# senikm/trpx

Hardware: AMD Instinct MI355X
Metric: frames/s (Terse encode + Prolix decode round trip, 512x512 uint16 stack, bit-exact vs CPU ref) (higher is better)
Workload: dtype u16

## Files before the change

### trpx_amd/csrc/encode_fused.hip

```cpp
#include <stddef.h>
#include <utility>
#include "codec_common.hpp"
#include "launchers.hpp"
#include "profile.hpp"
#include <stdlib.h>
#include <mutex>
#include <vector>

namespace trpx {

template <typename T> constexpr int sub_tiles() { return sizeof(T) <= 2 ? 4 : 5; }
template <typename T> constexpr int fused_occupancy() { return sizeof(T) <= 2 ? 8 : 4; }
[[maybe_unused]] constexpr uint64_t kWaitTicks = 25u * 1000u * 1000u;
struct SpinGuard {
    uint64_t t0 = 0;
    uint32_t spins = 0;
    __device__ __forceinline__ bool expired() {
#ifdef TRPX_FORCE_TIMEOUT
        return true;
#else
        if ((++spins & 63u) != 0u) return false;
        const uint64_t now = __builtin_amdgcn_s_memrealtime();
        if (t0 == 0) { t0 = now; return false; }
        return now - t0 > kWaitTicks;
#endif
    }
};

#ifdef TRPX_DIAGNOSTICS
#define TRPX_DIAG(a) ((a).debug)
#else
#define TRPX_DIAG(a) 0u
#endif

constexpr uint64_t kStInvalid = 0, kStAgg = 1, kStPrefix = 2;
constexpr uint32_t kGridY = 32768;
constexpr int kWmaxShift = 56;
constexpr uint64_t kBndHead = 1ull << 55;
constexpr uint64_t kHeadFlag = 1ull << 63, kTailFlag = 1ull << 62;
__device__ __forceinline__ uint64_t make_desc(uint64_t st, uint64_t v) { return (st << 62) | (v & ((1ull << 62) - 1)); }
__device__ __forceinline__ uint64_t desc_status(uint64_t d) { return d >> 62; }
__device__ __forceinline__ uint64_t desc_value(uint64_t d) { return d & ((1ull << 62) - 1); }

__device__ __forceinline__ uint64_t ld_desc(const uint64_t* p) {
    return __hip_atomic_load(p, __ATOMIC_RELAXED, __HIP_MEMORY_SCOPE_AGENT);
}
__device__ __forceinline__ void st_desc(uint64_t* p, uint64_t v) {
    __hip_atomic_store(p, v, __ATOMIC_RELAXED, __HIP_MEMORY_SCOPE_AGENT);
}

__device__ __forceinline__ uint64_t wave_sum64(uint64_t v) {
    const uint32_t l0 = (uint32_t)v & 0x1FFFFFu, l1 = (uint32_t)(v >> 21) & 0x1FFFFFu, l2 = (uint32_t)(v >> 42);
    const uint32_t s0 = (uint32_t)__builtin_amdgcn_readlane((int)wave_inclusive_scan(l0), 63);
    const uint32_t s1 = (uint32_t)__builtin_amdgcn_readlane((int)wave_inclusive_scan(l1), 63);
    const uint32_t s2 = (uint32_t)__builtin_amdgcn_readlane((int)wave_inclusive_scan(l2), 63);
    return (uint64_t)s0 + ((uint64_t)s1 << 21) + ((uint64_t)s2 << 42);
}

__device__ bool lookback(const uint64_t* __restrict__ desc, int64_t idx, int64_t lo, uint64_t* result) {
    const int lane = lane_id();
    uint64_t acc = 0;
    int64_t pos = idx - 1;
    while (pos >= lo) {
        const int64_t my = pos - lane;
        const bool in = my >= lo;
        uint64_t g = in ? 0ull : make_desc(kStPrefix, 0);
        uint32_t first_p = 64;
        SpinGuard guard;
        uint64_t need = ~0ull;
        for (;;) {
            if (desc_status(g) == kStInvalid && ((need >> lane) & 1ull)) g = ld_desc(desc + my);
            const uint64_t pmask = __ballot(desc_status(g) == kStPrefix);
            const uint64_t imask = __ballot(desc_status(g) == kStInvalid);
            first_p = pmask ? (uint32_t)__builtin_ctzll(pmask) : 64u;
            need = first_p >= 63u ? ~0ull : ((2ull << first_p) - 1ull);
            if ((imask & need) == 0) break;
            if (guard.expired()) return false;
            __builtin_amdgcn_s_sleep(2);
        }
        acc += wave_sum64((uint32_t)lane <= first_p ? desc_value(g) : 0ull);
        if (first_p < 64u) break;
        pos -= 64;
    }
    *result = acc;
    return true;
}

constexpr int kAccShift = 40;
constexpr uint32_t kAccLines = 2;
__host__ __device__ inline uint32_t fused_acc_lines(uint32_t tiles_per_frame) {
    const uint32_t k = (tiles_per_frame + 31u) / 32u;
    return k < 1u ? 1u : (k > kAccLines ? kAccLines : k);
}
constexpr uint64_t kPrefFlag = 1ull << 63;
__device__ bool lookback_frames(const uint64_t* __restrict__ acc_w, const uint64_t* __restrict__ pref_w, int64_t frame,
                                uint64_t tiles_per_frame, uint64_t* result, uint64_t stride, uint32_t n_acc) {
    const int lane = lane_id();
    uint64_t acc = 0;
    int64_t pos = frame - 1;
    while (pos >= 0) {
        const int64_t my = pos - lane;
        const bool in = my >= 0;
        uint64_t p = in ? 0ull : kPrefFlag, c = 0;
        uint32_t first_p = 64;
        SpinGuard guard;
        uint64_t need = ~0ull;
        bool complete = false;
        for (;;) {
            if (in && !(p & kPrefFlag) && !complete && ((need >> lane) & 1ull)) {
                p = ld_desc(pref_w + my * stride);
                c = ld_desc(acc_w + my * stride);
                for (uint32_t k = 1; k < n_acc; ++k) c += ld_desc(acc_w + my * stride + 16u * k);
                complete = (c >> kAccShift) == tiles_per_frame;
            }
            const uint64_t pmask = __ballot((p & kPrefFlag) != 0);
            const uint64_t cmask = __ballot(complete);
            first_p = pmask ? (uint32_t)__builtin_ctzll(pmask) : 64u;
            need = first_p >= 64u ? ~0ull : ((1ull << first_p) - 1ull);
            if ((~cmask & need) == 0) break;
            if (guard.expired()) return false;
            __builtin_amdgcn_s_sleep(2);
        }
        const uint64_t mine = (uint32_t)lane < first_p ? 1 + (c & ((1ull << kAccShift) - 1)) / 8
                                                       : ((uint32_t)lane == first_p ? p & ~kPrefFlag : 0ull);
        acc += wave_sum64(mine);
        if (first_p < 64u) break;
        pos -= 64;
    }
    *result = acc;
    return true;
}

template <typename T> struct Raw {
    static constexpr int bits = PixelTraits<T>::bits;
    static constexpr int per = 32 / bits;
    static constexpr int dw = kBlock / per;
};

template <typename T>
__device__ __forceinline__ uint32_t raw_field(const uint32_t (&raw)[Raw<T>::dw], int k) {
    constexpr int per = Raw<T>::per, bits = Raw<T>::bits;
    const uint32_t x = raw[k / per] >> ((k % per) * bits);
    return bits == 32 ? x : x & ((1u << (bits & 31)) - 1u);
}

template <typename T> struct QuadVec;
template <> struct QuadVec<uint8_t>  { typedef uint32_t type; };
template <> struct QuadVec<int8_t>   { typedef uint32_t type; };
template <> struct QuadVec<uint16_t> { typedef uint32_t type __attribute__((ext_vector_type(2))); };
template <> struct QuadVec<int16_t>  { typedef uint32_t type __attribute__((ext_vector_type(2))); };
template <> struct QuadVec<uint32_t> { typedef uint32_t type __attribute__((ext_vector_type(4))); };
template <> struct QuadVec<int32_t>  { typedef uint32_t type __attribute__((ext_vector_type(4))); };

template <typename T>
__device__ __forceinline__ void load_raw_nt(const T* __restrict__ p, uint32_t (&raw)[Raw<T>::dw]) {
    if constexpr (sizeof(T) == 2) {
        typedef uint32_t u4 __attribute__((ext_vector_type(4)));
        typedef uint32_t u2 __attribute__((ext_vector_type(2)));
        u4 lo; u2 hi;
        __builtin_memcpy(&lo, p, 16);
        __builtin_memcpy(&hi, reinterpret_cast<const char*>(p) + 16, 8);
        raw[0] = lo.x; raw[1] = lo.y; raw[2] = lo.z; raw[3] = lo.w; raw[4] = hi.x; raw[5] = hi.y;
        return;
    } else if constexpr (sizeof(T) == 1) {
        typedef uint32_t u3 __attribute__((ext_vector_type(3)));
        u3 x;
        __builtin_memcpy(&x, p, 12);
        raw[0] = x.x; raw[1] = x.y; raw[2] = x.z;
        return;
    }
    using V = typename QuadVec<T>::type;
    constexpr int q = Raw<T>::dw / 3;
    const V* src = reinterpret_cast<const V*>(p);
    union U { V vec; uint32_t x[q]; };
    U a, b, c;
    a.vec = src[0];
    b.vec = src[1];
    c.vec = src[2];
#pragma unroll
    for (int i = 0; i < q; ++i) { raw[i] = a.x[i]; raw[q + i] = b.x[i]; raw[2 * q + i] = c.x[i]; }
}
template <typename T>
__device__ __forceinline__ void load_raw_mis2(const T* __restrict__ p, uint32_t (&raw)[Raw<T>::dw]) {
    static_assert(sizeof(T) == 2, "16-bit pixels");
    typedef uint32_t u4 __attribute__((ext_vector_type(4)));
    typedef uint32_t u2 __attribute__((ext_vector_type(2)));
    const char* q = reinterpret_cast<const char*>(p) - 2;
    u4 lo; u2 hi; uint16_t last;
    __builtin_memcpy(&lo, q, 16);
    __builtin_memcpy(&hi, q + 16, 8);
    __builtin_memcpy(&last, q + 24, 2);
    raw[0] = __builtin_amdgcn_alignbit(lo.y, lo.x, 16); raw[1] = __builtin_amdgcn_alignbit(lo.z, lo.y, 16);
    raw[2] = __builtin_amdgcn_alignbit(lo.w, lo.z, 16); raw[3] = __builtin_amdgcn_alignbit(hi.x, lo.w, 16);
    raw[4] = __builtin_amdgcn_alignbit(hi.y, hi.x, 16); raw[5] = __builtin_amdgcn_alignbit((uint32_t)last, hi.y, 16);
}
template <typename T>
__device__ __forceinline__ void load_raw_partial(const T* __restrict__ p, int nb, uint32_t (&raw)[Raw<T>::dw]) {
    using UT = typename PixelTraits<T>::U;
#pragma unroll
    for (int i = 0; i < Raw<T>::dw; ++i) raw[i] = 0;
#pragma unroll
    for (int k = 0; k < kBlock; ++k)
        if (k < nb) raw[k / Raw<T>::per] |= (uint32_t)(UT)p[k] << ((k % Raw<T>::per) * Raw<T>::bits);
}

template <typename T>
__device__ __forceinline__ uint32_t raw_width(const uint32_t (&raw)[Raw<T>::dw]) {
    constexpr int bits = Raw<T>::bits;
    uint32_t m = 0;
    if (!PixelTraits<T>::is_signed) {
#pragma unroll
        for (int i = 0; i < Raw<T>::dw; ++i) m |= raw[i];
        if (bits == 16) m = (m | (m >> 16)) & 0xFFFFu;
        if (bits == 8) { m |= m >> 16; m = (m | (m >> 8)) & 0xFFu; }
    } else if (bits == 32) {
#pragma unroll
        for (int i = 0; i < Raw<T>::dw; ++i) {
            const uint32_t u = raw[i];
            m |= (int32_t)u < 0 ? 0u - u : u;
        }
    } else if (bits == 16) {
        typedef short s2 __attribute__((ext_vector_type(2)));
        typedef unsigned short us2 __attribute__((ext_vector_type(2)));
        uint32_t acc = 0;
#pragma unroll
        for (int i = 0; i < Raw<T>::dw; ++i) {
            union { uint32_t u; s2 v; us2 w; } x, n, y;
            x.u = raw[i];
            n.w = (us2)(0) - x.w;
            y.v = __builtin_elementwise_max(x.v, n.v);
            acc |= y.u;
        }
        m = (acc | (acc >> 16)) & 0xFFFFu;
    } else {
#pragma unroll
        for (int k = 0; k < kBlock; ++k) {
            const int32_t x = (int32_t)(int8_t)(raw[k / 4] >> ((k % 4) * 8));
            m |= (uint32_t)(x < 0 ? -x : x);
        }
    }
    return width_from_or<T>(m);
}

template <int ND>
__device__ __forceinline__ void lds_or_string(uint32_t* __restrict__ stage, uint32_t pos, uint32_t hv_top,
                                              const uint32_t* __restrict__ p) {
    const uint32_t d = (pos + 31u) >> 5, rs = (0u - pos) & 31u;
    const uint32_t xm = __builtin_amdgcn_alignbit(hv_top, 0u, rs);
    if (xm) atomicOr(&stage[d - 1], xm);
    if constexpr (ND == 0) {
        const uint32_t x0 = __builtin_amdgcn_alignbit(0u, hv_top, rs);
        if (x0) atomicOr(&stage[d], x0);
    } else {
        atomicOr(&stage[d], __builtin_amdgcn_alignbit(p[0], hv_top, rs));
#pragma unroll
        for (int j = 1; j < ND; ++j) {
            const uint32_t x = __builtin_amdgcn_alignbit(p[j], p[j - 1], rs);
            if (j >= ND - 1) atomicOr(&stage[d + j], x);
            else stage[d + j] = x;
        }
        const uint32_t x = __builtin_amdgcn_alignbit(0u, p[ND - 1], rs);
        if (x) atomicOr(&stage[d + ND], x);
    }
}

template <typename T, int W>
__device__ __forceinline__ void pack_payload_w(uint32_t* __restrict__ stage, uint32_t pos, uint32_t hv_top,
                                               const uint32_t (&raw)[Raw<T>::dw]) {
    constexpr int NB = kBlock * W;
    constexpr int ND = (NB + 31) / 32;
    constexpr int per = Raw<T>::per, bits = Raw<T>::bits;
    constexpr uint32_t MASK = W >= 32 ? 0xFFFFFFFFu : ((1u << (W & 31)) - 1u);
    uint32_t p[ND ? ND : 1];
#pragma unroll
    for (int j = 0; j < ND; ++j) p[j] = 0;
    if constexpr (W == 0) {
    } else if constexpr (bits == 16 && W < 16) {
        typedef unsigned short us2 __attribute__((ext_vector_type(2)));
        constexpr int L = (15 - W) / (2 * W) + 1;
        constexpr uint32_t kPairMask = MASK | (MASK << 16);
#pragma unroll
        for (int c = 0; c * L < kBlock / 2; ++c) {
            uint32_t acc = 0;
            int n_pairs = 0;
#pragma unroll
            for (int i = 0; i < L; ++i) {
                const int j = c * L + i;
                if (j < kBlock / 2) {
                    union { uint32_t u; us2 v; } x, k;
                    x.u = PixelTraits<T>::is_signed ? raw[j] & kPairMask : raw[j];
                    k.u = (1u << (2 * W * i)) | (1u << (2 * W * i + W + 16));
                    acc = __builtin_amdgcn_udot2(x.v, k.v, acc, false);
                    ++n_pairs;
                }
            }
            const int bit = 2 * W * L * c, nbits = 2 * W * n_pairs;
            p[bit >> 5] |= acc << (bit & 31);
            if ((bit & 31) + nbits > 32) p[(bit >> 5) + 1] |= acc >> (32 - (bit & 31));
        }
    } else if constexpr (bits == 16) {
#pragma unroll
        for (int j = 0; j < kBlock / 2; ++j) p[j] = raw[j];
    } else {
#pragma unroll
        for (int k = 0; k < kBlock; ++k) {
            const uint32_t u = (raw[k / per] >> ((k % per) * bits)) & MASK;
            const int bit = k * W;
            p[bit >> 5] |= u << (bit & 31);
            if ((bit & 31) + W > 32) p[(bit >> 5) + 1] |= u >> (32 - (bit & 31));
        }
    }
    lds_or_string<ND>(stage, pos, hv_top, p);
}

template <typename T, int LO, int HI>
struct PackDispatch {
    static __device__ __forceinline__ void run(uint32_t* stage, uint32_t pos, uint32_t hv_top, uint32_t w0,
                                               const uint32_t (&raw)[Raw<T>::dw]) {
        if constexpr (LO == HI) pack_payload_w<T, LO>(stage, pos, hv_top, raw);
        else {
            constexpr int MID = (LO + HI) / 2;
            if (w0 <= (uint32_t)MID) PackDispatch<T, LO, MID>::run(stage, pos, hv_top, w0, raw);
            else PackDispatch<T, MID + 1, HI>::run(stage, pos, hv_top, w0, raw);
        }
    }
};

template <typename T>
__device__ __forceinline__ void pack_payload_generic(uint32_t* __restrict__ stage, uint32_t pos, uint32_t w, int nb,
                                                     const uint32_t (&raw)[Raw<T>::dw]) {
    const uint32_t mask = w >= 32u ? 0xFFFFFFFFu : ((1u << w) - 1u);
#pragma unroll
    for (int k = 0; k < kBlock; ++k) {
        if (k < nb) {
            const uint64_t x = (uint64_t)(raw_field<T>(raw, k) & mask) << (pos & 31u);
            if ((uint32_t)x) atomicOr(&stage[pos >> 5], (uint32_t)x);
            if ((uint32_t)(x >> 32)) atomicOr(&stage[(pos >> 5) + 1], (uint32_t)(x >> 32));
            pos += w;
        }
    }
}

template <typename T> constexpr int fused_phase_rounds() { return (sub_tiles<T>() + 1) / 2; }
template <typename T>
constexpr int fused_stage_dwords() { return fused_phase_rounds<T>() * ((kThreads * max_block_bits<T>() + 31) / 32) + 12; }

struct FusedArgs {
    FrameGeom g;
    uint32_t n_frames;
    uint32_t tiles_per_frame;
    uint64_t out_capacity;
    uint64_t* tile_desc;
    uint64_t* tail_desc;
    uint64_t* bnd_pos;
    uint64_t* frame_acc;
    uint64_t* frame_pref;
    uint64_t* frame_base;
    uint32_t acc_stride;
    uint32_t n_acc;
    uint64_t* ws_tag;
    uint64_t expect_tag;
    uint64_t* frame_offsets;
    uint32_t* out32;
    uint32_t* status;
    uint8_t* idx_widths;
    uint64_t* idx_group_off;
    uint32_t debug;
    uint64_t* stamps;
};

typedef const char __attribute__((address_space(4)))* karg_ptr;
#define TRPX_KARG(kb, field) (*reinterpret_cast<const decltype(FusedArgs::field) __attribute__((address_space(4)))*>((kb) + 8 + offsetof(FusedArgs, field)))

template <typename T, bool MIS2>
__device__ __forceinline__ void encode_fused_body(const T* __restrict__ pixels, const FusedArgs& a) {
    constexpr int kSub = sub_tiles<T>();
    constexpr int kFusedTileBlocks = kSub * kThreads;
    constexpr int kStage = fused_stage_dwords<T>();
    constexpr int kStage4 = (kStage + 1 + 3) / 4;
    __shared__ __attribute__((aligned(16))) uint32_t s_stage_pad[4 * kStage4];
    uint32_t* const s_stage = s_stage_pad + 1;
    __shared__ uint32_t s_hdr[40];
    __shared__ uint32_t s_wtot[kSub * 4];
    __shared__ uint32_t s_wfl[kSub * 4];
    __shared__ uint64_t s_excl_bits;
    __shared__ uint64_t s_base_bytes;
    __shared__ uint32_t s_abort;
    __shared__ uint32_t s_carry;
    __shared__ uint32_t s_halo;

    const uint32_t tid = threadIdx.x;
#define TRPX_STAMP(slot) do { if ((TRPX_DIAG(a) & 4u) && threadIdx.x == 0) a.stamps[((uint64_t)(blockIdx.z * kGridY + blockIdx.y) * gridDim.x + blockIdx.x) * 8 + (slot)] = __builtin_amdgcn_s_memrealtime(); } while (0)
    TRPX_STAMP(0);
    const int lane = lane_id(), wave = wave_id();
    const FrameGeom g = a.g;
    const uint32_t t = blockIdx.x;
    const uint32_t frame = blockIdx.z * kGridY + blockIdx.y;
    const uint32_t n_frames = a.n_frames, tpf = a.tiles_per_frame;
    asm volatile("" :: "s"(g.n_values), "s"(g.n_blocks), "s"(n_frames), "s"(tpf), "s"(pixels));
    if (frame >= n_frames) return;
    const uint64_t tile = (uint64_t)frame * tpf + t;
    const bool last_tile_of_frame = t + 1 == tpf;
    if (tile == 0 && tid == 0) {
        karg_ptr kb0 = (karg_ptr)__builtin_amdgcn_kernarg_segment_ptr();
        uint64_t* const st64 = reinterpret_cast<uint64_t*>(TRPX_KARG(kb0, status));
#pragma unroll
        for (int i = 0; i < 4; ++i) st_desc(st64 + i, 0ull);
        const uint64_t want = TRPX_KARG(kb0, expect_tag);
        if (want != 0ull && ld_desc(TRPX_KARG(kb0, ws_tag)) != want) atomicMax(&TRPX_KARG(kb0, status)[0], 7u);
        asm volatile("s_waitcnt vmcnt(0)" ::: "memory");
    }
    const T* fp = pixels + (uint64_t)frame * g.n_values;
    const uint32_t b0 = t * kFusedTileBlocks;

    uint32_t v[kSub][Raw<T>::dw];
    uint32_t w[kSub], up[kSub], len[kSub], inc[kSub];
    int nb[kSub];
    const bool has_full = g.n_values >= (uint64_t)kBlock;
    const uint64_t max_first = has_full ? g.n_values - kBlock : 0;
    uint32_t h[Raw<T>::dw];
    [[maybe_unused]] const bool mis2 = MIS2 && ((uintptr_t)fp & 2u) != 0u && frame != 0u;
    if (has_full) {
        bool loaded = false;
        if constexpr (MIS2 && sizeof(T) == 2) {
            if (mis2) {
#pragma unroll
                for (int r = 0; r < kSub; ++r) {
                    const uint64_t first = (uint64_t)(b0 + r * kThreads + tid) * kBlock;
                    load_raw_mis2<T>(fp + (first < max_first ? first : max_first), v[r]);
                }
                loaded = true;
            }
        }
        if (!loaded) {
#pragma unroll
            for (int r = 0; r < kSub; ++r) {
                const uint64_t first = (uint64_t)(b0 + r * kThreads + tid) * kBlock;
                load_raw_nt<T>(fp + (first < max_first ? first : max_first), v[r]);
            }
        }
        if (wave == 0) load_raw_nt<T>(fp + (uint64_t)(b0 ? b0 - 1 : 0) * kBlock, h);
        else {
#pragma unroll
            for (int i = 0; i < Raw<T>::dw; ++i) h[i] = 0u;
        }
    } else {
#pragma unroll
        for (int r = 0; r < kSub; ++r)
#pragma unroll
            for (int i = 0; i < Raw<T>::dw; ++i) v[r][i] = 0u;
#pragma unroll
        for (int i = 0; i < Raw<T>::dw; ++i) h[i] = 0u;
    }
    const uint32_t nb_tail = (uint32_t)(g.n_values - (uint64_t)(g.n_blocks - 1) * kBlock);
#pragma unroll
    for (int r = 0; r < kSub; ++r) {
        const uint32_t b1 = b0 + r * kThreads + tid + 1u;
        nb[r] = b1 < g.n_blocks ? kBlock : (b1 == g.n_blocks ? (int)nb_tail : 0);
    }
    if (tid == 0) s_abort = 0;
    if (tid <= 32u) s_hdr[tid] = header_val(tid, tid + 1u) << (32u - header_len(tid, tid + 1u));
    {
        typedef uint32_t u4 __attribute__((ext_vector_type(4)));
        u4* z = reinterpret_cast<u4*>(s_stage_pad);
#pragma unroll
        for (int i = 0; i < (kStage4 + kThreads - 1) / kThreads; ++i)
            if (i * kThreads + (int)tid < kStage4) z[i * kThreads + tid] = (u4)(0u);
    }
    uint32_t pv[Raw<T>::dw];
#pragma unroll
    for (int i = 0; i < Raw<T>::dw; ++i) pv[i] = 0u;
    if (last_tile_of_frame && g.n_values % kBlock) {
        const uint32_t bp = g.n_blocks - 1;
        if (bp >= b0 && (bp - b0) % kThreads == tid) load_raw_partial<T>(fp + (uint64_t)bp * kBlock, (int)(g.n_values % kBlock), pv);
    }
    TRPX_STAMP(7);
    uint32_t w_part = 0u;
    if (last_tile_of_frame && g.n_values % kBlock) w_part = raw_width<T>(pv);
    if (wave == 0) {
        const uint32_t hw0 = b0 > 0 ? raw_width<T>(h) : 0u;
        if (lane == 0) s_halo = hw0;
    }
    uint32_t wmax = 0;
    uint32_t hlr[kSub];
#pragma unroll
    for (int r = 0; r < kSub; ++r) {
        w[r] = nb[r] == kBlock ? raw_width<T>(v[r]) : (nb[r] ? w_part : 0u);
        wmax = w[r] > wmax ? w[r] : wmax;
        if (a.idx_widths && nb[r]) a.idx_widths[(uint64_t)frame * g.n_blocks + b0 + r * kThreads + tid] = (uint8_t)w[r];
        up[r] = (uint32_t)__builtin_amdgcn_update_dpp(0, (int)w[r], 0x138, 0xf, 0xf, false);
        hlr[r] = header_len(w[r], up[r]);
        len[r] = nb[r] ? (lane ? hlr[r] : 0u) + (uint32_t)nb[r] * w[r] : 0u;
    }
    static_assert(kWave * max_block_bits<T>() < 65536, "packed scan needs 16-bit wave totals");
#pragma unroll
    for (int r = 0; r + 1 < kSub; r += 2) {
        const uint32_t two = wave_inclusive_scan(len[r] | (len[r + 1] << 16));
        inc[r] = two & 0xFFFFu;
        inc[r + 1] = two >> 16;
    }
    if (kSub & 1) inc[kSub - 1] = wave_inclusive_scan(len[kSub - 1]);
    const uint32_t wmax_wave = wave_max(wmax);
#pragma unroll
    for (int r = 0; r < kSub; ++r) {
        const uint32_t w_first = (uint32_t)__builtin_amdgcn_readfirstlane((int)w[r]);
        const uint32_t v_first = (uint32_t)__builtin_amdgcn_readfirstlane(nb[r]);
        if (lane == 63) {
            s_wtot[r * 4 + wave] = inc[r];
            s_wfl[r * 4 + wave] = w_first | (w[r] << 8) | ((v_first ? 1u : 0u) << 16) | (r == 0 ? wmax_wave << 24 : 0u);
        }
    }
    TRPX_STAMP(5);
    __syncthreads();
    TRPX_STAMP(1);

    const uint32_t tile_halo = s_halo;
    uint32_t rb[kSub + 1];
    uint32_t off[kSub];
    uint32_t meta[kSub];
    {
        uint32_t tot = 0, h0 = 0, wprev = 0;
        if (lane < kSub * 4) {
            const uint32_t wfl = s_wfl[lane];
            wprev = lane == 0 ? tile_halo : (s_wfl[lane - 1] >> 8) & 0xFFu;
            h0 = (wfl >> 16) & 1u ? header_len(wfl & 0xFFu, wprev) : 0u;
            tot = s_wtot[lane] + h0;
        }
        const uint32_t incl = wave_inclusive_scan(tot);
        const uint32_t excl = incl - tot;
        const uint32_t hw = h0 | (wprev << 8);
        const int swave = __builtin_amdgcn_readfirstlane(wave);
#pragma unroll
        for (int r = 0; r < kSub; ++r) {
            rb[r] = (uint32_t)__builtin_amdgcn_readlane((int)excl, r * 4);
            const uint32_t pb = (uint32_t)__builtin_amdgcn_readlane((int)excl, r * 4 + swave);
            const uint32_t ph = (uint32_t)__builtin_amdgcn_readlane((int)hw, r * 4 + swave);
            off[r] = pb + (lane ? (ph & 0xFFu) : 0u) + inc[r] - len[r];
            const uint32_t wp_r = lane ? up[r] : ph >> 8;
            const uint32_t hl_r = lane ? hlr[r] : (ph & 0xFFu);
            meta[r] = w[r] | (wp_r << 8) | (hl_r << 16) | (nb[r] == kBlock ? 1u << 24 : 0u) | (nb[r] ? 1u << 25 : 0u);
        }
        rb[kSub] = (uint32_t)__builtin_amdgcn_readlane((int)incl, kSub * 4 - 1);
    }
    const uint32_t tile_total = rb[kSub];

    if (tid == 0 && !(TRPX_DIAG(a) & 1u)) {
        st_desc(a.tile_desc + tile, make_desc(t == 0 ? kStPrefix : kStAgg, tile_total));
        __hip_atomic_fetch_add(a.frame_acc + (uint64_t)frame * a.acc_stride + 16u * (t % a.n_acc), (1ull << kAccShift) | tile_total, __ATOMIC_RELAXED, __HIP_MEMORY_SCOPE_AGENT);
    }
    constexpr int kPhaseRounds = fused_phase_rounds<T>();
    constexpr uint32_t kCapBits = (uint32_t)kPhaseRounds * kThreads * max_block_bits<T>();
    const bool two_phase = tile_total > kCapBits;
    uint64_t p0 = 0, p_end = 0;
    uint64_t img_p0 = 0;
    uint32_t bias = 0;
    bool writable = false;
#define TRPX_WSTAMP(slot) do { if ((TRPX_DIAG(a) & 8u) && lane == 0 && tile < 4096) a.stamps[tile * 32 + wave * 8 + (slot)] = __builtin_amdgcn_s_memrealtime(); } while (0)
    auto pack_round = [&](auto rc) {
        constexpr int r = decltype(rc)::value;
        const uint32_t pos = off[r] - bias;
        const uint32_t mr = meta[r];
        const uint32_t hl = (mr >> 16) & 0xFFu;
        const uint32_t wr = mr & 0xFFu;
        const uint32_t hv_top = wr == ((mr >> 8) & 0xFFu) ? 0x80000000u : s_hdr[wr];
        const bool full = (mr >> 24) & 1u;
        if (((mr >> 25) & 1u) && !full) {
            const uint64_t hx = (uint64_t)(hv_top >> (32u - hl)) << (pos & 31u);
            atomicOr(&s_stage[pos >> 5], (uint32_t)hx);
            if ((uint32_t)(hx >> 32)) atomicOr(&s_stage[(pos >> 5) + 1], (uint32_t)(hx >> 32));
            if (wr) pack_payload_generic<T>(s_stage, pos + hl, wr, (int)nb_tail, pv);
        }
        uint64_t todo = __ballot(full);
        while (todo) {
            const int l0 = __builtin_ctzll(todo);
            const uint32_t w0 = (uint32_t)__builtin_amdgcn_readlane((int)wr, l0);
            const bool mine = full && wr == w0;
            uint32_t wd = w0;
            asm volatile("" : "+s"(wd));
#pragma unroll
            for (int i = 0; i < Raw<T>::dw; ++i) asm volatile("" : "+v"(v[r][i]));
            if (mine) PackDispatch<T, 0, PixelTraits<T>::bits>::run(s_stage_pad, pos + hl, hv_top, wd, v[r]);
            todo &= ~__ballot(mine);
        }
        TRPX_WSTAMP(1 + r);
    };
    auto look_back = [&]() {
        if (wave == 0) {
            uint64_t excl = 0;
            bool ok = true;
            if (TRPX_DIAG(a) & 1u) excl = (uint64_t)t * 40000u;
            else if (t != 0) {
                ok = lookback(a.tile_desc, (int64_t)tile, (int64_t)(tile - t), &excl);
                if (ok && lane == 0) st_desc(a.tile_desc + tile, make_desc(kStPrefix, excl + tile_total));
            }
            if (lane == 0) { s_excl_bits = excl; if (!ok) s_abort = 1; }
            TRPX_STAMP(2);
        } else if (wave == 1) {
            uint64_t base = 0;
            bool ok = true;
            if (TRPX_DIAG(a) & 1u) base = (uint64_t)frame * 120000u;
            else if (t == 0) {
                ok = lookback_frames(a.frame_acc, a.frame_pref, (int64_t)frame, a.tiles_per_frame, &base, a.acc_stride, a.n_acc);
                if (ok && lane == 0) st_desc(a.frame_base + (uint64_t)frame * 16, kPrefFlag | base);
            } else {
                uint64_t vb = 0;
                SpinGuard guard;
                for (;;) {
                    vb = ld_desc(a.frame_base + (uint64_t)frame * 16);
                    if (vb & kPrefFlag) break;
                    if (guard.expired()) { ok = false; break; }
                    __builtin_amdgcn_s_sleep(2);
                }
                base = vb & ~kPrefFlag;
            }
            if (lane == 0) { s_base_bytes = base; if (!ok) s_abort = 1; }
        }
    };
    auto place_tile = [&]() -> bool {
        karg_ptr kb = (karg_ptr)__builtin_amdgcn_kernarg_segment_ptr();
        asm volatile("" : "+s"(kb));
        const bool aborted = s_abort != 0;
        const uint64_t excl_bits = s_excl_bits, base_bytes = s_base_bytes;
        const uint64_t frame_size = 1 + (excl_bits + tile_total) / 8;
        if (last_tile_of_frame && tid == 0 && !aborted) {
            st_desc(TRPX_KARG(kb, frame_pref) + (uint64_t)frame * TRPX_KARG(kb, acc_stride), kPrefFlag | (base_bytes + frame_size));
            TRPX_KARG(kb, frame_offsets)[frame + 1] = base_bytes + frame_size;
            if (frame == 0) TRPX_KARG(kb, frame_offsets)[0] = 0;
            if (frame + 1 == TRPX_KARG(kb, n_frames) && align_up(base_bytes + frame_size, 4) > TRPX_KARG(kb, out_capacity))
                atomicMax(&TRPX_KARG(kb, status)[0], 3u);
        }
        if (aborted) {
            if (tid == 0) atomicMax(&TRPX_KARG(kb, status)[0], 7u);
            return false;
        }
        if (TRPX_KARG(kb, idx_group_off) && tid < (uint32_t)kSub && b0 + tid * kThreads < g.n_blocks) {
            uint32_t rbv = 0;
#pragma unroll
            for (int r = 0; r < kSub; ++r) rbv = tid == (uint32_t)r ? rb[r] : rbv;
            TRPX_KARG(kb, idx_group_off)[(uint64_t)frame * g.n_tiles + (uint64_t)t * kSub + tid] = excl_bits + rbv;
        }
        p0 = 8 * base_bytes + excl_bits;
        p_end = last_tile_of_frame ? 8 * (base_bytes + frame_size) : p0 + tile_total;
        writable = align_up((p_end + 7) / 8, 4) <= TRPX_KARG(kb, out_capacity);
        img_p0 = p0;
        return true;
    };
    auto flush = [&](bool first, bool carry_out, uint64_t q_end) {
        karg_ptr kb = (karg_ptr)__builtin_amdgcn_kernarg_segment_ptr();
        asm volatile("" : "+s"(kb));
        uint32_t* const out32 = TRPX_KARG(kb, out32);
        uint64_t* const tail_desc = TRPX_KARG(kb, tail_desc);
        const uint32_t s0 = (uint32_t)(img_p0 & 31), sh = (32u - s0) & 31u;
        const bool head_pending = s0 != 0;
        const uint64_t d_first = img_p0 >> 5, d_last = q_end >> 5;
        const int32_t k_first = head_pending ? -1 : 0;
        const uint32_t n_out = (uint32_t)(d_last - d_first);
        const bool completed_first = d_last > d_first;
        const bool is_last_tile = tile + 1 == (uint64_t)TRPX_KARG(kb, n_frames) * TRPX_KARG(kb, tiles_per_frame);
        if (tid == 0) {
            const int32_t kt = k_first + (int32_t)n_out;
            const uint32_t tail_bits = (q_end & 31) ? __builtin_amdgcn_alignbit(s_stage[kt + 1], s_stage[kt], sh) : 0u;
            if (head_pending) {
                const uint32_t head_bits = __builtin_amdgcn_alignbit(s_stage[0], 0u, sh);
                __hip_atomic_fetch_or(tail_desc + tile, kHeadFlag | head_bits, __ATOMIC_RELAXED, __HIP_MEMORY_SCOPE_AGENT);
            }
            if (first) {
                uint32_t wm = 0;
#pragma unroll
                for (int i = 0; i < 4; ++i) wm = (s_wfl[i] >> 24) > wm ? (s_wfl[i] >> 24) : wm;
                TRPX_KARG(kb, bnd_pos)[tile] = (head_pending ? d_first | kBndHead : 0ull) | ((uint64_t)wm << kWmaxShift);
            }
            if (carry_out) s_carry = tail_bits;
            else if ((q_end & 31) != 0 && (completed_first || !head_pending)) {
                if (is_last_tile) { if (writable) __builtin_nontemporal_store(tail_bits, out32 + d_last); }
                else __hip_atomic_fetch_or(tail_desc + tile + 1, kTailFlag | tail_bits, __ATOMIC_RELAXED, __HIP_MEMORY_SCOPE_AGENT);
            }
        }
        if (writable) {
            typedef uint32_t u4 __attribute__((ext_vector_type(4)));
            uint32_t al = (0u - ((uint32_t)((uintptr_t)out32 >> 2) + (uint32_t)d_first)) & 3u;
            if (head_pending && al == 0) al = 4;
            al = al < n_out ? al : n_out;
            const uint32_t n4 = (n_out - al) >> 2, rest0 = al + 4 * n4;
            if (tid < al + (n_out - rest0)) {
                const uint32_t j = tid < al ? tid : rest0 + (tid - al);
                if (!(j == 0 && head_pending)) {
                    const int32_t k = k_first + (int32_t)j;
                    __builtin_nontemporal_store(__builtin_amdgcn_alignbit(s_stage[k + 1], s_stage[k], sh), out32 + d_first + j);
                }
            }
            const uint32_t kk0 = (uint32_t)(k_first + 1) + al;
            const uint32_t m = kk0 & 3u;
            const u4* pad4 = reinterpret_cast<const u4*>(s_stage_pad) + (kk0 >> 2);
            u4* dst = reinterpret_cast<u4*>(out32 + d_first + al);
#define TRPX_FLUSH_GROUPS(M)                                                                                   \
            for (uint32_t gq = tid; gq < n4; gq += kThreads) {                                                 \
                const u4 A = pad4[gq], B = pad4[gq + 1];                                                       \
                const uint32_t e[8] = {A.x, A.y, A.z, A.w, B.x, B.y, B.z, B.w};                                \
                u4 x;                                                                                          \
                x.x = __builtin_amdgcn_alignbit(e[M + 1], e[M + 0], sh);                                       \
                x.y = __builtin_amdgcn_alignbit(e[M + 2], e[M + 1], sh);                                       \
                x.z = __builtin_amdgcn_alignbit(e[M + 3], e[M + 2], sh);                                       \
                x.w = __builtin_amdgcn_alignbit(e[M + 4], e[M + 3], sh);                                       \
                __builtin_nontemporal_store(x, dst + gq);                                                      \
            }
            if (m == 0) { TRPX_FLUSH_GROUPS(0) } else if (m == 1) { TRPX_FLUSH_GROUPS(1) }
            else if (m == 2) { TRPX_FLUSH_GROUPS(2) } else { TRPX_FLUSH_GROUPS(3) }
#undef TRPX_FLUSH_GROUPS
        }
    };

    TRPX_WSTAMP(0);
    [&]<int... R>(std::integer_sequence<int, R...>) { (pack_round(std::integral_constant<int, R>{}), ...); }(std::make_integer_sequence<int, kPhaseRounds>{});
    if (two_phase) {
        look_back();
        __syncthreads();
        if (!place_tile()) return;
        flush(true, true, p0 + rb[kPhaseRounds]);
        const uint64_t d_last = (p0 + rb[kPhaseRounds]) >> 5;
        __syncthreads();
        {
            typedef uint32_t u4 __attribute__((ext_vector_type(4)));
            u4* z = reinterpret_cast<u4*>(s_stage_pad);
            for (int i = (int)tid; i < kStage4; i += kThreads) z[i] = (u4)(0u);
        }
        __syncthreads();
        if (tid == 0 && s_carry) atomicOr(&s_stage[0], s_carry);
        img_p0 = 32 * d_last;
        bias = (uint32_t)(img_p0 - p0);
    }
    [&]<int... R>(std::integer_sequence<int, R...>) { (pack_round(std::integral_constant<int, kPhaseRounds + R>{}), ...); }(std::make_integer_sequence<int, kSub - kPhaseRounds>{});
    if (!two_phase) look_back();
    __syncthreads();
    TRPX_STAMP(3);
    if (!two_phase && !place_tile()) return;
    flush(!two_phase, false, p_end);
    TRPX_STAMP(4);
    if ((TRPX_DIAG(a) & 4u) && tid == 0) { uint32_t xcc; asm volatile("s_getreg_b32 %0, hwreg(HW_REG_XCC_ID)" : "=s"(xcc)); a.stamps[tile * 8 + 6] = xcc; }
}

template <typename T>
__global__ __launch_bounds__(kThreads, fused_occupancy<T>()) void k_encode_fused(const T* __restrict__ pixels, FusedArgs a) {
    encode_fused_body<T, false>(pixels, a);
}
template <typename T>
__global__ __launch_bounds__(kThreads, fused_occupancy<T>() - 1) void k_encode_fused_mis2(const T* __restrict__ pixels, FusedArgs a) {
    encode_fused_body<T, true>(pixels, a);
}

__global__ __launch_bounds__(kThreads) void k_stitch(uint64_t* __restrict__ tile_desc, uint64_t* __restrict__ xw, const uint64_t* __restrict__ pos,
                                                     uint64_t n_tiles, uint64_t* __restrict__ frame_words, uint64_t n_frame_words,
                                                     uint64_t* __restrict__ ws_tag, uint64_t tag, uint32_t* __restrict__ out32,
                                                     uint64_t out_capacity, uint32_t* __restrict__ status) {
    __shared__ uint32_t s_max[4];
    const uint64_t b = (uint64_t)blockIdx.x * kThreads + threadIdx.x;
    constexpr uint64_t kPosMask = kBndHead - 1;
    const bool in = b < n_tiles;
    const uint32_t st0 = __hip_atomic_load(&status[0], __ATOMIC_RELAXED, __HIP_MEMORY_SCOPE_AGENT);
    const uint64_t pw = in ? pos[b] : 0ull;
    const uint64_t pb = in && b > 0 ? pos[b - 1] : 0ull;
    const uint64_t xb = in ? xw[b] : 0ull;
    const bool failed = st0 != 0u;
    const uint32_t wm = wave_max(failed ? 0u : (uint32_t)(pw >> kWmaxShift));
    if (lane_id() == 0) s_max[wave_id()] = wm;
    __syncthreads();
    if (threadIdx.x == 0) {
        uint32_t m = s_max[0];
        for (int i = 1; i < 4; ++i) m = s_max[i] > m ? s_max[i] : m;
        if (m) atomicMax(&status[1], m);
    }
    for (uint64_t i = b; i < n_frame_words; i += (uint64_t)gridDim.x * kThreads) frame_words[i] = 0ull;
    if (b == 0 && ws_tag) ws_tag[0] = tag;
    if (b >= n_tiles) return;
    tile_desc[b] = 0ull;
    if (failed || b == 0) { xw[b] = 0ull; return; }
    if (!(pw & kBndHead)) { xw[b] = 0ull; return; }
    const uint64_t d = pw & kPosMask;
    if (b > 1 && (pb & kBndHead) && (pb & kPosMask) == d) return;
    uint32_t acc = (uint32_t)xb;
    xw[b] = 0ull;
    for (uint64_t k = b + 1; k < n_tiles; ++k) {
        const uint64_t pk = pos[k];
        if (!((pk & kBndHead) && (pk & kPosMask) == d)) break;
        acc |= (uint32_t)xw[k];
        xw[k] = 0ull;
    }
    if (4 * d + 4 <= out_capacity) out32[d] = acc;
}

template <typename T>
static uint32_t fused_tiles_per_frame(const FrameGeom& g) {
    constexpr uint32_t tb = sub_tiles<T>() * kThreads;
    return (g.n_blocks + tb - 1) / tb;
}

size_t fused_workspace_bytes(const FrameGeom& g, size_t n_frames) {
    const size_t tpf = ((size_t)g.n_blocks + 2 * kThreads - 1) / (2 * kThreads);
    return align_up(8 * (3 * n_frames * tpf + 16 * ((size_t)kAccLines + 1) * n_frames + 1), 256) + 64 * n_frames * tpf;
}

namespace {
struct CleanSig {
    uint32_t elem, tiles_per_frame, n_frames, n_blocks;
    bool operator==(const CleanSig& o) const { return elem == o.elem && tiles_per_frame == o.tiles_per_frame && n_frames == o.n_frames && n_blocks == o.n_blocks; }
};
struct CleanWs { int device; const void* ptr; CleanSig sig; uint64_t tag; };
std::mutex g_clean_mu;
std::vector<CleanWs> g_clean;
uint64_t g_next_tag = 0x5452505800000001ull;
}
void fused_ws_forget(const void* lo, size_t bytes, const void* keep) {
    std::lock_guard<std::mutex> lk(g_clean_mu);
    const char* a = static_cast<const char*>(lo);
    for (size_t i = 0; i < g_clean.size();) {
        const char* p = static_cast<const char*>(g_clean[i].ptr);
        if (p != keep && (!lo || (p >= a && p < a + bytes))) { g_clean[i] = g_clean.back(); g_clean.pop_back(); } else ++i;
    }
}

template <typename T>
static hipError_t launch_fused_t(const EncodeArgs& e, void* ws, hipStream_t st) {
    FusedArgs a;
    a.g = e.geom;
    a.n_frames = e.n_frames;
    a.tiles_per_frame = fused_tiles_per_frame<T>(e.geom);
    a.out_capacity = e.out_capacity;
    const size_t tiles = (size_t)e.n_frames * a.tiles_per_frame;
    a.tile_desc = static_cast<uint64_t*>(ws);
    a.tail_desc = a.tile_desc + tiles;
    a.bnd_pos = a.tail_desc + tiles;
    a.n_acc = fused_acc_lines(a.tiles_per_frame);
    a.acc_stride = 16u * a.n_acc;
    a.frame_acc = a.bnd_pos + tiles;
    a.frame_pref = a.frame_acc + 1;
    a.frame_base = a.frame_acc + (size_t)a.acc_stride * e.n_frames;
    a.frame_offsets = e.frame_offsets;
    a.out32 = reinterpret_cast<uint32_t*>(e.out);
    a.status = e.status;
    a.idx_widths = e.idx_widths;
    a.idx_group_off = e.idx_group_off;
    const size_t frame_words = 16 * ((size_t)a.n_acc + 1) * e.n_frames;
    uint64_t* const frame_words_base = a.frame_acc;
    a.ws_tag = frame_words_base + frame_words;
    a.stamps = reinterpret_cast<uint64_t*>(static_cast<char*>(ws) + align_up(8 * (3 * tiles + frame_words + 1), 256));
#ifdef TRPX_DIAGNOSTICS
    a.debug = getenv("TRPX_FUSED_DEBUG") ? (uint32_t)atoi(getenv("TRPX_FUSED_DEBUG")) : 0u;
#else
    a.debug = 0u;
#endif
    hipStreamCaptureStatus cap = hipStreamCaptureStatusNone;
    if (hipStreamIsCapturing(st, &cap) != hipSuccess) { (void)hipGetLastError(); cap = hipStreamCaptureStatusActive; }
    const bool capturing = cap != hipStreamCaptureStatusNone;
    int device = -1;
    (void)hipGetDevice(&device);
    const CleanSig sig{(uint32_t)sizeof(T), a.tiles_per_frame, e.n_frames, e.geom.n_blocks};
    uint64_t expect = 0, tag = 0;
    if (!capturing) {
        std::lock_guard<std::mutex> lk(g_clean_mu);
        tag = g_next_tag++;
        for (size_t i = 0; i < g_clean.size(); ++i)
            if (g_clean[i].device == device && g_clean[i].ptr == ws) {
                if (g_clean[i].sig == sig) expect = g_clean[i].tag;
                g_clean[i] = g_clean.back(); g_clean.pop_back();
                break;
            }
    }
    a.expect_tag = expect;
    Profiler& prof = profiler();
    prof.begin();
    prof.mark(st);
    if (expect == 0)
        hipLaunchKernelGGL(k_zero_words<0>, dim3(256), dim3(kThreads), 0, st, static_cast<uint64_t*>(ws),
                           (uint64_t)(3 * tiles + frame_words + (capturing ? 0 : 1)), reinterpret_cast<uint64_t*>(e.status), (uint64_t)4);
    prof.mark(st);
    const dim3 grid(a.tiles_per_frame, e.n_frames < kGridY ? e.n_frames : kGridY, (e.n_frames + kGridY - 1) / kGridY);
    bool mis2 = false;
    if constexpr (sizeof(T) == 2) mis2 = (((uintptr_t)e.pixels & 2u) != 0u || (e.geom.n_values & 1u) != 0u) && e.n_frames > 1u;
    if constexpr (sizeof(T) == 2) {
        if (mis2) hipLaunchKernelGGL((k_encode_fused_mis2<T>), grid, dim3(kThreads), 0, st, static_cast<const T*>(e.pixels), a);
    }
    if (!mis2) hipLaunchKernelGGL((k_encode_fused<T>), grid, dim3(kThreads), 0, st, static_cast<const T*>(e.pixels), a);
    prof.mark(st);
    hipLaunchKernelGGL(k_stitch, dim3((uint32_t)((tiles + kThreads - 1) / kThreads)), dim3(kThreads), 0, st,
                       a.tile_desc, a.tail_desc, static_cast<const uint64_t*>(a.bnd_pos), (uint64_t)tiles, frame_words_base, (uint64_t)frame_words,
                       capturing ? static_cast<uint64_t*>(nullptr) : a.ws_tag, tag, a.out32, (uint64_t)e.out_capacity, a.status);
    prof.mark(st);
    const hipError_t err = hipGetLastError();
    if (err == hipSuccess && !capturing) {
        std::lock_guard<std::mutex> lk(g_clean_mu);
        if (g_clean.size() >= 64) g_clean.erase(g_clean.begin());
        g_clean.push_back(CleanWs{device, ws, sig, tag});
    }
    return err;
}

hipError_t launch_encode_fused(int dtype, const EncodeArgs& e, void* ws, hipStream_t st) {
    return for_pixel_type(dtype, [&]<class T>() { return launch_fused_t<T>(e, ws, st); });
}

}
```

Before: 3.731 million.

## Specialize fused encode front-end for interior tiles without bounds checks

Wraps the tile front-end (loads, width computation, scans, tile-level prefix) in a lambda that gets compiled twice: once for interior tiles, where every block is full, and once for the general path. The interior version drops the per-block clamping and nb bookkeeping, uses scalar-base address arithmetic, and computes header length and bit length with cheaper constant forms. It also pads the shared staging buffer to a multiple of the thread count so the zeroing loop runs unguarded, and the index-write check becomes a single want_idx flag. The cost is larger code and higher register pressure from two instantiations, plus more LDS when the padding is enabled.

```diff
diff --git a/trpx_amd/csrc/encode_fused.hip b/trpx_amd/csrc/encode_fused.hip
--- a/trpx_amd/csrc/encode_fused.hip
+++ b/trpx_amd/csrc/encode_fused.hip
@@ -378,7 +378,9 @@
     constexpr int kFusedTileBlocks = kSub * kThreads;
     constexpr int kStage = fused_stage_dwords<T>();
     constexpr int kStage4 = (kStage + 1 + 3) / 4;
-    __shared__ __attribute__((aligned(16))) uint32_t s_stage_pad[4 * kStage4];
+    constexpr int kStage4Up = (kStage4 + kThreads - 1) / kThreads * kThreads;
+    constexpr int kStageAlloc4 = !MIS2 && fused_occupancy<T>() * (16 * kStage4Up + 512) <= 160 * 1024 ? kStage4Up : kStage4;
+    __shared__ __attribute__((aligned(16))) uint32_t s_stage_pad[4 * kStageAlloc4];
     uint32_t* const s_stage = s_stage_pad + 1;
     __shared__ uint32_t s_hdr[40];
     __shared__ uint32_t s_wtot[kSub * 4];
@@ -414,134 +416,186 @@
     const uint32_t b0 = t * kFusedTileBlocks;
 
     uint32_t v[kSub][Raw<T>::dw];
-    uint32_t w[kSub], up[kSub], len[kSub], inc[kSub];
-    int nb[kSub];
-    const bool has_full = g.n_values >= (uint64_t)kBlock;
-    const uint64_t max_first = has_full ? g.n_values - kBlock : 0;
-    uint32_t h[Raw<T>::dw];
-    [[maybe_unused]] const bool mis2 = MIS2 && ((uintptr_t)fp & 2u) != 0u && frame != 0u;
-    if (has_full) {
-        bool loaded = false;
-        if constexpr (MIS2 && sizeof(T) == 2) {
-            if (mis2) {
-#pragma unroll
-                for (int r = 0; r < kSub; ++r) {
-                    const uint64_t first = (uint64_t)(b0 + r * kThreads + tid) * kBlock;
-                    load_raw_mis2<T>(fp + (first < max_first ? first : max_first), v[r]);
-                }
-                loaded = true;
-            }
-        }
-        if (!loaded) {
-#pragma unroll
-            for (int r = 0; r < kSub; ++r) {
-                const uint64_t first = (uint64_t)(b0 + r * kThreads + tid) * kBlock;
-                load_raw_nt<T>(fp + (first < max_first ? first : max_first), v[r]);
-            }
-        }
-        if (wave == 0) load_raw_nt<T>(fp + (uint64_t)(b0 ? b0 - 1 : 0) * kBlock, h);
-        else {
-#pragma unroll
-            for (int i = 0; i < Raw<T>::dw; ++i) h[i] = 0u;
-        }
-    } else {
-#pragma unroll
-        for (int r = 0; r < kSub; ++r)
-#pragma unroll
-            for (int i = 0; i < Raw<T>::dw; ++i) v[r][i] = 0u;
-#pragma unroll
-        for (int i = 0; i < Raw<T>::dw; ++i) h[i] = 0u;
-    }
-    const uint32_t nb_tail = (uint32_t)(g.n_values - (uint64_t)(g.n_blocks - 1) * kBlock);
-#pragma unroll
-    for (int r = 0; r < kSub; ++r) {
-        const uint32_t b1 = b0 + r * kThreads + tid + 1u;
-        nb[r] = b1 < g.n_blocks ? kBlock : (b1 == g.n_blocks ? (int)nb_tail : 0);
-    }
-    if (tid == 0) s_abort = 0;
-    if (tid <= 32u) s_hdr[tid] = header_val(tid, tid + 1u) << (32u - header_len(tid, tid + 1u));
-    {
-        typedef uint32_t u4 __attribute__((ext_vector_type(4)));
-        u4* z = reinterpret_cast<u4*>(s_stage_pad);
-#pragma unroll
-        for (int i = 0; i < (kStage4 + kThreads - 1) / kThreads; ++i)
-            if (i * kThreads + (int)tid < kStage4) z[i * kThreads + tid] = (u4)(0u);
-    }
     uint32_t pv[Raw<T>::dw];
-#pragma unroll
-    for (int i = 0; i < Raw<T>::dw; ++i) pv[i] = 0u;
-    if (last_tile_of_frame && g.n_values % kBlock) {
-        const uint32_t bp = g.n_blocks - 1;
-        if (bp >= b0 && (bp - b0) % kThreads == tid) load_raw_partial<T>(fp + (uint64_t)bp * kBlock, (int)(g.n_values % kBlock), pv);
-    }
-    TRPX_STAMP(7);
-    uint32_t w_part = 0u;
-    if (last_tile_of_frame && g.n_values % kBlock) w_part = raw_width<T>(pv);
-    if (wave == 0) {
-        const uint32_t hw0 = b0 > 0 ? raw_width<T>(h) : 0u;
-        if (lane == 0) s_halo = hw0;
-    }
-    uint32_t wmax = 0;
-    uint32_t hlr[kSub];
-#pragma unroll
-    for (int r = 0; r < kSub; ++r) {
-        w[r] = nb[r] == kBlock ? raw_width<T>(v[r]) : (nb[r] ? w_part : 0u);
-        wmax = w[r] > wmax ? w[r] : wmax;
-        if (a.idx_widths && nb[r]) a.idx_widths[(uint64_t)frame * g.n_blocks + b0 + r * kThreads + tid] = (uint8_t)w[r];
-        up[r] = (uint32_t)__builtin_amdgcn_update_dpp(0, (int)w[r], 0x138, 0xf, 0xf, false);
-        hlr[r] = header_len(w[r], up[r]);
-        len[r] = nb[r] ? (lane ? hlr[r] : 0u) + (uint32_t)nb[r] * w[r] : 0u;
-    }
-    static_assert(kWave * max_block_bits<T>() < 65536, "packed scan needs 16-bit wave totals");
-#pragma unroll
-    for (int r = 0; r + 1 < kSub; r += 2) {
-        const uint32_t two = wave_inclusive_scan(len[r] | (len[r + 1] << 16));
-        inc[r] = two & 0xFFFFu;
-        inc[r + 1] = two >> 16;
-    }
-    if (kSub & 1) inc[kSub - 1] = wave_inclusive_scan(len[kSub - 1]);
-    const uint32_t wmax_wave = wave_max(wmax);
-#pragma unroll
-    for (int r = 0; r < kSub; ++r) {
-        const uint32_t w_first = (uint32_t)__builtin_amdgcn_readfirstlane((int)w[r]);
-        const uint32_t v_first = (uint32_t)__builtin_amdgcn_readfirstlane(nb[r]);
-        if (lane == 63) {
-            s_wtot[r * 4 + wave] = inc[r];
-            s_wfl[r * 4 + wave] = w_first | (w[r] << 8) | ((v_first ? 1u : 0u) << 16) | (r == 0 ? wmax_wave << 24 : 0u);
-        }
-    }
-    TRPX_STAMP(5);
-    __syncthreads();
-    TRPX_STAMP(1);
-
-    const uint32_t tile_halo = s_halo;
     uint32_t rb[kSub + 1];
     uint32_t off[kSub];
     uint32_t meta[kSub];
-    {
-        uint32_t tot = 0, h0 = 0, wprev = 0;
-        if (lane < kSub * 4) {
-            const uint32_t wfl = s_wfl[lane];
-            wprev = lane == 0 ? tile_halo : (s_wfl[lane - 1] >> 8) & 0xFFu;
-            h0 = (wfl >> 16) & 1u ? header_len(wfl & 0xFFu, wprev) : 0u;
-            tot = s_wtot[lane] + h0;
-        }
-        const uint32_t incl = wave_inclusive_scan(tot);
-        const uint32_t excl = incl - tot;
-        const uint32_t hw = h0 | (wprev << 8);
-        const int swave = __builtin_amdgcn_readfirstlane(wave);
+    const uint32_t nb_tail = (uint32_t)(g.n_values - (uint64_t)(g.n_blocks - 1) * kBlock);
+    const bool want_idx = a.idx_widths != nullptr;
+    const bool interior = !MIS2 && (uint64_t)b0 + kFusedTileBlocks + (nb_tail != (uint32_t)kBlock ? 1u : 0u) <= (uint64_t)g.n_blocks;
+    auto front = [&](auto interior_c) {
+        constexpr bool kInterior = decltype(interior_c)::value;
+        uint32_t w[kSub], up[kSub], len[kSub], inc[kSub];
+        int nb[kSub];
+        uint32_t h[Raw<T>::dw];
+        if constexpr (kInterior) {
+            constexpr uint32_t kBlockBytes = kBlock * sizeof(T);
+            const char* const tile_bytes = reinterpret_cast<const char*>(fp) + (uint64_t)b0 * kBlockBytes;
+            const uint32_t lane_bytes = kBlockBytes == 24u ? (tid << 4) + (tid << 3) : tid * kBlockBytes;
+#pragma unroll
+            for (int r = 0; r < kSub; ++r) {
+                const char* round_bytes = tile_bytes + (uint32_t)r * kThreads * kBlockBytes;
+                asm volatile("" : "+s"(round_bytes));
+                load_raw_nt<T>(reinterpret_cast<const T*>(round_bytes + lane_bytes), v[r]);
+                nb[r] = kBlock;
+            }
+            if (wave == 0) load_raw_nt<T>(fp + (uint64_t)(b0 ? b0 - 1 : 0) * kBlock, h);
+            else {
+#pragma unroll
+                for (int i = 0; i < Raw<T>::dw; ++i) h[i] = 0u;
+            }
+        } else {
+        const bool has_full = g.n_values >= (uint64_t)kBlock;
+        const uint64_t max_first = has_full ? g.n_values - kBlock : 0;
+        [[maybe_unused]] const bool mis2 = MIS2 && ((uintptr_t)fp & 2u) != 0u && frame != 0u;
+        if (has_full) {
+            bool loaded = false;
+            if constexpr (MIS2 && sizeof(T) == 2) {
+                if (mis2) {
+#pragma unroll
+                    for (int r = 0; r < kSub; ++r) {
+                        const uint64_t first = (uint64_t)(b0 + r * kThreads + tid) * kBlock;
+                        load_raw_mis2<T>(fp + (first < max_first ? first : max_first), v[r]);
+                    }
+                    loaded = true;
+                }
+            }
+            if (!loaded) {
+#pragma unroll
+                for (int r = 0; r < kSub; ++r) {
+                    const uint64_t first = (uint64_t)(b0 + r * kThreads + tid) * kBlock;
+                    load_raw_nt<T>(fp + (first < max_first ? first : max_first), v[r]);
+                }
+            }
+            if (wave == 0) load_raw_nt<T>(fp + (uint64_t)(b0 ? b0 - 1 : 0) * kBlock, h);
+            else {
+#pragma unroll
+                for (int i = 0; i < Raw<T>::dw; ++i) h[i] = 0u;
+            }
+        } else {
+#pragma unroll
+            for (int r = 0; r < kSub; ++r)
+#pragma unroll
+                for (int i = 0; i < Raw<T>::dw; ++i) v[r][i] = 0u;
+#pragma unroll
+            for (int i = 0; i < Raw<T>::dw; ++i) h[i] = 0u;
+        }
 #pragma unroll
         for (int r = 0; r < kSub; ++r) {
-            rb[r] = (uint32_t)__builtin_amdgcn_readlane((int)excl, r * 4);
-            const uint32_t pb = (uint32_t)__builtin_amdgcn_readlane((int)excl, r * 4 + swave);
-            const uint32_t ph = (uint32_t)__builtin_amdgcn_readlane((int)hw, r * 4 + swave);
-            off[r] = pb + (lane ? (ph & 0xFFu) : 0u) + inc[r] - len[r];
-            const uint32_t wp_r = lane ? up[r] : ph >> 8;
-            const uint32_t hl_r = lane ? hlr[r] : (ph & 0xFFu);
-            meta[r] = w[r] | (wp_r << 8) | (hl_r << 16) | (nb[r] == kBlock ? 1u << 24 : 0u) | (nb[r] ? 1u << 25 : 0u);
-        }
-        rb[kSub] = (uint32_t)__builtin_amdgcn_readlane((int)incl, kSub * 4 - 1);
-    }
+            const uint32_t b1 = b0 + r * kThreads + tid + 1u;
+            nb[r] = b1 < g.n_blocks ? kBlock : (b1 == g.n_blocks ? (int)nb_tail : 0);
+        }
+        }
+        if (tid == 0) s_abort = 0;
+        if (tid <= 32u) s_hdr[tid] = header_val(tid, tid + 1u) << (32u - header_len(tid, tid + 1u));
+        {
+            typedef uint32_t u4 __attribute__((ext_vector_type(4)));
+            u4* z = reinterpret_cast<u4*>(s_stage_pad);
+            if constexpr (MIS2) {
+#pragma unroll
+                for (int i = 0; i < (kStageAlloc4 + kThreads - 1) / kThreads; ++i)
+                    if (i * kThreads + (int)tid < kStageAlloc4) z[i * kThreads + tid] = (u4)(0u);
+            } else {
+#pragma unroll
+                for (int i = 0; i < kStageAlloc4 / kThreads; ++i) z[i * kThreads + tid] = (u4)(0u);
+                if constexpr (kStageAlloc4 % kThreads != 0)
+                    if ((kStageAlloc4 / kThreads) * kThreads + (int)tid < kStageAlloc4) z[(kStageAlloc4 / kThreads) * kThreads + tid] = (u4)(0u);
+            }
+        }
+        uint32_t w_part = 0u;
+        if constexpr (!kInterior) {
+#pragma unroll
+        for (int i = 0; i < Raw<T>::dw; ++i) pv[i] = 0u;
+        if (last_tile_of_frame && g.n_values % kBlock) {
+            const uint32_t bp = g.n_blocks - 1;
+            if (bp >= b0 && (bp - b0) % kThreads == tid) load_raw_partial<T>(fp + (uint64_t)bp * kBlock, (int)(g.n_values % kBlock), pv);
+        }
+        }
+        TRPX_STAMP(7);
+        if constexpr (!kInterior)
+        if (last_tile_of_frame && g.n_values % kBlock) w_part = raw_width<T>(pv);
+        if (wave == 0) {
+            const uint32_t hw0 = b0 > 0 ? raw_width<T>(h) : 0u;
+            if (lane == 0) s_halo = hw0;
+        }
+        uint32_t wmax = 0;
+        uint32_t hlr[kSub];
+#pragma unroll
+        for (int r = 0; r < kSub; ++r) {
+            w[r] = nb[r] == kBlock ? raw_width<T>(v[r]) : (nb[r] ? w_part : 0u);
+            wmax = w[r] > wmax ? w[r] : wmax;
+            up[r] = (uint32_t)__builtin_amdgcn_update_dpp(0, (int)w[r], 0x138, 0xf, 0xf, false);
+            if constexpr (kInterior) {
+                hlr[r] = 1u;
+                if (w[r] != up[r]) hlr[r] = explicit_header_len(w[r]);
+                len[r] = (lane ? hlr[r] : 0u) + (w[r] << 3) + (w[r] << 2);
+            } else {
+                hlr[r] = header_len(w[r], up[r]);
+                len[r] = nb[r] ? (lane ? hlr[r] : 0u) + (uint32_t)nb[r] * w[r] : 0u;
+            }
+        }
+        if (want_idx) {
+            uint8_t* const iw = a.idx_widths + ((uint64_t)frame * g.n_blocks + b0);
+#pragma unroll
+            for (int r = 0; r < kSub; ++r)
+                if (kInterior || nb[r]) iw[(uint32_t)(r * kThreads) + tid] = (uint8_t)w[r];
+        }
+        static_assert(kWave * max_block_bits<T>() < 65536, "packed scan needs 16-bit wave totals");
+#pragma unroll
+        for (int r = 0; r + 1 < kSub; r += 2) {
+            const uint32_t two = wave_inclusive_scan(len[r] | (len[r + 1] << 16));
+            inc[r] = two & 0xFFFFu;
+            inc[r + 1] = two >> 16;
+        }
+        if (kSub & 1) inc[kSub - 1] = wave_inclusive_scan(len[kSub - 1]);
+        const uint32_t wmax_wave = wave_max(wmax);
+        uint32_t wfl[kSub];
+#pragma unroll
+        for (int r = 0; r < kSub; ++r) {
+            const uint32_t w_first = (uint32_t)__builtin_amdgcn_readfirstlane((int)w[r]);
+            wfl[r] = w_first | (r == 0 ? wmax_wave << 24 : 0u);
+            if constexpr (!kInterior) wfl[r] |= (__builtin_amdgcn_readfirstlane(nb[r]) ? 1u : 0u) << 16;
+        }
+        if (lane == 63) {
+#pragma unroll
+            for (int r = 0; r < kSub; ++r) {
+                s_wtot[r * 4 + wave] = inc[r];
+                s_wfl[r * 4 + wave] = wfl[r] | (w[r] << 8);
+            }
+        }
+        TRPX_STAMP(5);
+        __syncthreads();
+        TRPX_STAMP(1);
+
+        const uint32_t tile_halo = s_halo;
+        {
+            uint32_t tot = 0, h0 = 0, wprev = 0;
+            if (lane < kSub * 4) {
+                const uint32_t wfl = s_wfl[lane];
+                wprev = lane == 0 ? tile_halo : (s_wfl[lane - 1] >> 8) & 0xFFu;
+                h0 = kInterior || ((wfl >> 16) & 1u) ? header_len(wfl & 0xFFu, wprev) : 0u;
+                tot = s_wtot[lane] + h0;
+            }
+            const uint32_t incl = wave_inclusive_scan(tot);
+            const uint32_t excl = incl - tot;
+            const uint32_t hw = h0 | (wprev << 8);
+            const int swave = __builtin_amdgcn_readfirstlane(wave);
+#pragma unroll
+            for (int r = 0; r < kSub; ++r) {
+                rb[r] = (uint32_t)__builtin_amdgcn_readlane((int)excl, r * 4);
+                const uint32_t pb = (uint32_t)__builtin_amdgcn_readlane((int)excl, r * 4 + swave);
+                const uint32_t ph = (uint32_t)__builtin_amdgcn_readlane((int)hw, r * 4 + swave);
+                off[r] = pb + (lane ? (ph & 0xFFu) : 0u) + inc[r] - len[r];
+                const uint32_t wp_r = lane ? up[r] : ph >> 8;
+                const uint32_t hl_r = lane ? hlr[r] : (ph & 0xFFu);
+                meta[r] = w[r] | (wp_r << 8) | (hl_r << 16) | (nb[r] == kBlock ? 1u << 24 : 0u) | (nb[r] ? 1u << 25 : 0u);
+            }
+            rb[kSub] = (uint32_t)__builtin_amdgcn_readlane((int)incl, kSub * 4 - 1);
+        }
+    };
+    if constexpr (MIS2) front(std::false_type{});
+    else if (interior) front(std::true_type{});
+    else front(std::false_type{});
     const uint32_t tile_total = rb[kSub];
 
     if (tid == 0 && !(TRPX_DIAG(a) & 1u)) {
@@ -633,11 +687,14 @@
             if (tid == 0) atomicMax(&TRPX_KARG(kb, status)[0], 7u);
             return false;
         }
-        if (TRPX_KARG(kb, idx_group_off) && tid < (uint32_t)kSub && b0 + tid * kThreads < g.n_blocks) {
-            uint32_t rbv = 0;
-#pragma unroll
-            for (int r = 0; r < kSub; ++r) rbv = tid == (uint32_t)r ? rb[r] : rbv;
-            TRPX_KARG(kb, idx_group_off)[(uint64_t)frame * g.n_tiles + (uint64_t)t * kSub + tid] = excl_bits + rbv;
+        if (want_idx) {
+            uint64_t* const group_off = TRPX_KARG(kb, idx_group_off);
+            if (tid < (uint32_t)kSub && b0 + tid * kThreads < g.n_blocks) {
+                uint32_t rbv = 0;
+#pragma unroll
+                for (int r = 0; r < kSub; ++r) rbv = tid == (uint32_t)r ? rb[r] : rbv;
+                group_off[(uint64_t)frame * g.n_tiles + (uint64_t)t * kSub + tid] = excl_bits + rbv;
+            }
         }
         p0 = 8 * base_bytes + excl_bits;
         p_end = last_tile_of_frame ? 8 * (base_bytes + frame_size) : p0 + tile_total;
```

Result: faster. 3.791 million, median of 6 (+1.6%).
